# Jingliang-Duan/DSAC-v2

Measured on AMD Instinct MI355X. Metric: DSAC-T gradient steps/sec, batch=256 Humanoid (obs376/act17), higher is better.
Workload: dtype f32

## Files before the change

### dsac-v2_amd/csrc/dsact_chain.h

```cpp
#pragma once
#include "dsact_kernels.h"

namespace dsact {

#ifndef DSACT_TILE_NAP
#define DSACT_TILE_NAP 24
#endif
constexpr int kChMaxL = 4;
#ifndef DSACT_KPD
#define DSACT_KPD 16
#endif
constexpr int kPD = DSACT_KPD;

#ifdef DSACT_TIMELINE
#define CTL(buf, k) do { if ((buf) && threadIdx.x == 0 && blockIdx.x < 1024) (buf)[blockIdx.x * 16 + (k)] = (long long)__builtin_readcyclecounter(); } while (0)
#define CTLR(buf, k) do { if ((buf) && threadIdx.x == 0 && blockIdx.x < 1024) (buf)[blockIdx.x * 16 + (k)] = (long long)__builtin_amdgcn_s_memrealtime(); } while (0)
#define CTLV(buf, k, v) do { if ((buf) && threadIdx.x == 0 && blockIdx.x < 1024) (buf)[blockIdx.x * 16 + (k)] = (long long)(v); } while (0)
#else
#define CTL(buf, k) do {} while (0)
#define CTLR(buf, k) do {} while (0)
#define CTLV(buf, k, v) do {} while (0)
#endif


struct WStr { f32x4 b[kPD]; };

__device__ __forceinline__ void stream_prologue(WStr& ws, const float* cur, int s_lo, int lane4) {
#pragma unroll
  for (int u = 0; u < kPD; ++u) ws.b[u] = gload4(cur + (size_t)(s_lo + u) * 256 + lane4);
}

template <int RG>
__device__ __forceinline__ void gemm44_seg(WStr& ws, const float* cur, int s_lo, int s_hi, const float* nxt, int nxt_s0,
                                           bool has_nxt, const float* lds, int xs, int ld, int lane4, f32x4 (&acc)[RG][2]) {
  f32x4 a0[RG], a1[RG];
#pragma unroll
  for (int g = 0; g < RG; ++g) a0[g] = *(const f32x4*)(lds + xs + 4 * g * ld + 4 * s_lo);
  for (int s0 = s_lo; s0 < s_hi; s0 += kPD) {
    const float* src = s0 + kPD < s_hi ? cur + (size_t)(s0 + kPD) * 256
                                       : (has_nxt ? nxt + (size_t)nxt_s0 * 256 : cur + (size_t)s_lo * 256);
#pragma unroll
    for (int u = 0; u < kPD; ++u) {
      const int s = s0 + u;
#pragma unroll
      for (int g = 0; g < RG; ++g) {
        if (u & 1) a0[g] = *(const f32x4*)(lds + xs + 4 * g * ld + 4 * (s + 1));
        else a1[g] = *(const f32x4*)(lds + xs + 4 * g * ld + 4 * (s + 1));
      }
#pragma unroll
      for (int e = 0; e < 4; ++e) {
#pragma unroll
        for (int g = 0; g < RG; ++g)
          acc[g][e & 1] = __builtin_amdgcn_mfma_f32_4x4x1f32((u & 1) ? a1[g][e] : a0[g][e], ws.b[u][e], acc[g][e & 1], 0, 0, 0);
        if (e == 1) __builtin_amdgcn_sched_barrier(0);
      }
      ws.b[u] = gload4(src + (size_t)u * 256 + lane4);
      __builtin_amdgcn_sched_barrier(0);
    }
  }
}

template <int NTO_MAX>
struct NarrowFrags { f32x4 w[NTO_MAX][4]; };

template <int NTO_MAX>
__device__ __forceinline__ void narrow_load(NarrowFrags<NTO_MAX>& f, const float* wf, int C, int nto, int wave, int lane4) {
#pragma unroll
  for (int t = 0; t < NTO_MAX; ++t) {
    if (t < nto) {
#pragma unroll
      for (int c = 0; c < 4; ++c) f.w[t][c] = gload4(wf + ((size_t)t * C + (size_t)wave * 4 + c) * 256 + lane4);
    }
  }
}
template <int NTO_MAX>
__device__ __forceinline__ void narrow_mma(const NarrowFrags<NTO_MAX>& f, int nto, int wave, float* lds, int xs, int red, int lane) {
  f32x4 a[4];
#pragma unroll
  for (int c = 0; c < 4; ++c) a[c] = *(const f32x4*)(lds + xs + 16 * (wave * 4 + c));
#pragma unroll
  for (int t = 0; t < NTO_MAX; ++t) {
    if (t < nto) {
      f32x4 acc = {0.f, 0.f, 0.f, 0.f};
#pragma unroll
      for (int c = 0; c < 4; ++c)
#pragma unroll
        for (int e = 0; e < 4; ++e) acc = __builtin_amdgcn_mfma_f32_16x16x4f32(f.w[t][c][e], a[c][e], acc, 0, 0, 0);
      *(f32x4*)(lds + red + ((wave * NTO_MAX + t) * 64 + lane) * 4) = acc;
    }
  }
}
template <int NTO_MAX, int NW>
__device__ __forceinline__ float narrow_get(const float* lds, int red, int m, int n) {
  const int t = n >> 4, ln = (((n & 15) >> 2) << 4) + m, e = n & 3;
  float s = lds[red + ((0 * NTO_MAX + t) * 64 + ln) * 4 + e];
#pragma unroll
  for (int w = 1; w < NW; ++w) s += lds[red + ((w * NTO_MAX + t) * 64 + ln) * 4 + e];
  return s;
}

template <int TPR>
__device__ __forceinline__ float rowN_sum(float v) {
  v += dpp_mov<0xB1>(v);
  v += dpp_mov<0x4E>(v);
  if (TPR >= 8) v += dpp_mov<0x141>(v);
  if (TPR >= 16) v += dpp_mov<0x140>(v);
  if (TPR >= 32) { float a, b; swap16(v, a, b); v = a + b; }
  if (TPR >= 64) { float a, b; swap32(v, a, b); v = a + b; }
  return v;
}

__device__ __forceinline__ bool chain_decode(int b, int n_units, int n_slices, int& unit, int& slice) {
  const int rep = n_units >= 5 ? 1 : (n_units >= 3 ? 2 : (n_units == 2 ? 4 : 8));
  const int xcd = b & 7, rnd = b >> 3;
  if (xcd >= n_units * rep) return false;
  unit = xcd % n_units;
  slice = rnd * rep + xcd / n_units;
  return slice < n_slices;
}
inline int chain_grid(int n_units, int n_slices) {
  const int rep = n_units >= 5 ? 1 : (n_units >= 3 ? 2 : (n_units == 2 ? 4 : 8));
  return 8 * ((n_slices + rep - 1) / rep);
}
struct XcdMap { int unit[8], base[8], stride[8]; };
inline XcdMap xcd_map_uniform(int n_units) {
  XcdMap m;
  const int rep = n_units >= 5 ? 1 : (n_units >= 3 ? 2 : (n_units == 2 ? 4 : 8));
  for (int x = 0; x < 8; ++x) {
    const bool on = x < n_units * rep;
    m.unit[x] = on ? x % n_units : -1; m.base[x] = on ? x / n_units : 0; m.stride[x] = rep;
  }
  return m;
}
inline XcdMap xcd_map_shares(int n_units, const int* share) {
  XcdMap m;
  int x = 0;
  for (int u = 0; u < n_units; ++u)
    for (int k = 0; k < share[u] && x < 8; ++k, ++x) { m.unit[x] = u; m.base[x] = k; m.stride[x] = share[u]; }
  for (; x < 8; ++x) { m.unit[x] = -1; m.base[x] = 0; m.stride[x] = 1; }
// ... 365 lines not shown
  int s_obs, s_act;
  int v1_stats;
  const float* act_scale; const float* act_center; float lo_ls, hi_ls;
  long long* timeline;
  int* spin_timeout;
  int debug_withhold;
  const long long* tagp;
  int tpad;
  int x0_lds;
};


__device__ __forceinline__ void stores_acked_barrier() {
  asm volatile("s_waitcnt vmcnt(0) lgkmcnt(0)\n\ts_barrier" ::: "memory");
}
__device__ __forceinline__ void chain_publish(int* flag, int value = 1) {
  if (!flag) return;
  stores_acked_barrier();
  if (threadIdx.x == 0) __hip_atomic_store(flag, value, __ATOMIC_RELAXED, __HIP_MEMORY_SCOPE_AGENT);
}
__device__ __forceinline__ void chain_wait(const int* f0, const int* f1, int* timeout) {
  if (threadIdx.x == 0) {
    int spins = 0;
    for (;;) {
      const int a0 = f0 ? __hip_atomic_load(f0, __ATOMIC_RELAXED, __HIP_MEMORY_SCOPE_AGENT) : 1;
      const int a1 = f1 ? __hip_atomic_load(f1, __ATOMIC_RELAXED, __HIP_MEMORY_SCOPE_AGENT) : 1;
      if (a0 && a1) break;
      if (++spins > (1 << 17)) { if (timeout) *timeout = 1; break; }
      __builtin_amdgcn_s_sleep(16);
    }
  }
  __syncthreads();
}

constexpr int kArriveStride = 64;
__device__ __forceinline__ void pack_store4(float* p, const f32x4& v, int agent) {
  if (agent) asm volatile("global_store_dwordx4 %0, %1, off sc1" : : "v"(p), "v"(v) : "memory");
  else nt_store4(p, v);
}
__device__ __forceinline__ void hand_store(float* p, float v, int agent) {
  if (agent) st_agent(p, v); else *p = v;
}
__device__ __forceinline__ void chain_arrive(int* cnt) {
  if (!cnt) return;
  stores_acked_barrier();
  if (threadIdx.x < 8) __hip_atomic_fetch_add(cnt + threadIdx.x * kArriveStride, 1, __ATOMIC_RELAXED, __HIP_MEMORY_SCOPE_AGENT);
}
struct ArriveWait {
  const int* cnt; int need; int* timeout;
  long long* tl = nullptr;
  int quick = 0;
  __device__ __forceinline__ void operator()() const {
    if (threadIdx.x == 0) {
      const int* c = cnt + ((int)blockIdx.x & 7) * kArriveStride;
      int spins = 0;
      while (__hip_atomic_load(c, __ATOMIC_RELAXED, __HIP_MEMORY_SCOPE_AGENT) < need) {
        if (++spins > (1 << 17)) { if (timeout) *timeout = 1; break; }
        if (quick) __builtin_amdgcn_s_sleep(4); else __builtin_amdgcn_s_sleep(DSACT_TILE_NAP);
      }
    }
    asm volatile("s_barrier" ::: "memory");
    CTLR(tl, 13);
  }
};

__device__ __forceinline__ bool fwd_decode(const FwdArgs& a, int b, int& unit, int& slice) {
  const int x = b & 7;
  unit = a.map.unit[x];
  if (unit < 0) return false;
  slice = a.map.base[x] + a.map.stride[x] * (b >> 3);
  return slice < a.u[unit].n_slices;
}
inline int fwd_grid(const FwdArgs& a) {
  int rounds = 0;
  for (int x = 0; x < 8; ++x) {
    if (a.map.unit[x] < 0) continue;
    const int n = a.u[a.map.unit[x]].n_slices - a.map.base[x];
    const int r = n > 0 ? (n + a.map.stride[x] - 1) / a.map.stride[x] : 0;
    rounds = r > rounds ? r : rounds;
  }
  return 8 * rounds;
}

template <int NW, int RG, bool GA = false, typename AT = FwdArgs, typename UT = FwdUnit, bool WARM = false>
__device__ __forceinline__ void chain_fwd_body(const AT& a, const UT& u, int unit, int slice, float* lds, int warm_idx = 0, int warm_cnt = 0) {
  constexpr int W = 64 * NW, SH = W / 4, R = 4 * RG, NTHR = 64 * NW, TPR = NTHR / R;
  int* const done_flag = (u.done && !(a.debug_withhold && unit == 0 && slice == 0)) ? u.done + slice : nullptr;
  const int tid = threadIdx.x, lane = tid & 63;
  const int wave = __builtin_amdgcn_readfirstlane(tid >> 6);
  const int lane4 = lane * 4;
  const int n = 64 * wave + lane;
  const int row0 = slice * R;
  const int L = a.L, F = a.F, A = a.A;
  const int S0 = a.s_obs + u.s_act;
  const int head = u.head & HEAD_KIND, twin = u.head & (HEAD_TWIN_FIRST | HEAD_TWIN_SECOND);
  const int c_out = ((u.head >> 8) & 0xff) ? ((u.head >> 8) & 0xff) : W / 16;
  const int oact = GA ? head_out_act(u.head) : 0;
  const ChainLds S = chain_lds(4 * (a.s_obs + a.s_act), W, R);
  const int xin = S.off_in, red = S.off_red;
  CTL(a.timeline, 0);
  CTLR(a.timeline, 14);
  const bool do_obs = u.seg != SEG_ACT_FROM_SAVED;
  const bool do_act = u.seg != SEG_OBS_ONLY && u.s_act > 0;
  WStr ws;
  const float* w0 = u.wf[0] + (size_t)wave * (S0 + a.tpad) * 256;
  stream_prologue(ws, w0, do_obs ? 0 : a.s_obs, lane4);
  constexpr int NWARM = 4;
  float wt[NWARM] = {0.f, 0.f, 0.f, 0.f};
  if (WARM) {
    const int n0 = NW * S0 * 8, nh = NW * SH * 8;
    const int nhead = head == HEAD_NONE ? 0 : (head == HEAD_POLICY ? (2 * A + 15) >> 4 : 1) * (W / 16) * 8;
    const int total = warm_cnt > 0 ? n0 + (L - 1) * nh + nhead : 0;
    const int share = (total + warm_cnt - 1) / (warm_cnt > 0 ? warm_cnt : 1);
    const int lo = warm_idx * share, hi = lo + share < total ? lo + share : total;
    const float* wb[kChMaxL + 1];
#pragma unroll
    for (int l = 0; l <= kChMaxL; ++l) wb[l] = u.wf[l <= L ? l : L];
#pragma unroll
    for (int q = 0; q < NWARM; ++q) {
      int i = lo + tid + q * NTHR;
      i = i < hi ? i : lo;
      const float* base = wb[0];
      int off = i;
#pragma unroll
      for (int l = 1; l <= kChMaxL; ++l) {
        const int start = n0 + (l - 1) * nh;
        const bool in = l <= L && i >= start;
        base = in ? wb[l] : base;
        off = in ? i - start : off;
      }
      wt[q] = *(const __attribute__((address_space(1))) float*)(base + (size_t)off * 32);
    }
    __builtin_amdgcn_sched_barrier(0);
  }
  float bq[kChMaxL];
#pragma unroll
  for (int l = 0; l < kChMaxL; ++l) bq[l] = u.bias[l < L ? l : 0][n];
  const int mr = tid / TPR, jr = tid % TPR;
  constexpr int NQ = (32 + TPR - 1) / TPR;
  float pre_eps[NQ], pre_bmu[NQ], pre_braw[NQ], pre_s[NQ], pre_c[NQ];
#pragma unroll
  for (int q = 0; q < NQ; ++q) { pre_eps[q] = 0.f; pre_bmu[q] = 0.f; pre_braw[q] = 0.f; pre_s[q] = 1.f; pre_c[q] = 0.f; }
  if (head == HEAD_POLICY) {
#pragma unroll
    for (int q = 0; q < NQ; ++q) {
      const int d = jr + q * TPR;
      if (d < A) {
        pre_eps[q] = u.eps[(size_t)(row0 + mr) * A + d];
        pre_bmu[q] = u.bias[L][d]; pre_braw[q] = u.bias[L][A + d];
        pre_s[q] = a.act_scale[d]; pre_c[q] = a.act_center[d];
      }
    }
  } else if (head == HEAD_Q && jr == 0) {
    pre_bmu[0] = u.bias[L][0]; pre_braw[0] = u.bias[L][1];
  }
  const bool pairs_in = (u.late_wait & HW_PAIRS_IN) != 0, pairs_out = (u.late_wait & HW_PAIRS_OUT) != 0;
  const unsigned tag = (pairs_in || pairs_out) ? (unsigned)(*a.tagp) + 1u : 0u;
  const bool head_wait = (u.late_wait & HW_HEAD) != 0;
  const int* const flag0 = (pairs_in || head_wait) ? nullptr : u.wait0;
  const bool waits = flag0 || u.wait1 || pairs_in;
  const bool late = waits && (u.late_wait & HW_LATE) && u.seg != SEG_ACT_FROM_SAVED && u.s_act > 0;
  if ((flag0 || u.wait1) && !late)
    chain_wait(flag0 ? flag0 + row0 / u.wait_rows0 : nullptr, u.wait1 ? u.wait1 + row0 / u.wait_rows1 : nullptr, a.spin_timeout);
  f32x4 zi[RG];
  if (u.seg == SEG_ACT_FROM_SAVED) {
#pragma unroll
    for (int g = 0; g < RG; ++g)
#pragma unroll
      for (int r = 0; r < 4; ++r) zi[g][r] = ld_agent(u.zinit + (size_t)(row0 + 4 * g + r) * W + n);
  }
  auto stage_act = [&]() {
    const int Fp = 4 * a.s_obs;
    if (pairs_in) {
      const unsigned long long* hp = (const unsigned long long*)u.wait0;
      const int per_row = 4 * u.s_act;
      for (int e = tid; e < R * per_row; e += NTHR) {
        const int r = e / per_row, k = e % per_row;
        float v = 0.0f;
        if (k < A) {
          const unsigned long long* src = hp + (size_t)(row0 + r) * 32 + k;
          unsigned long long pv = __hip_atomic_load(src, __ATOMIC_RELAXED, __HIP_MEMORY_SCOPE_AGENT);
          int spins = 0;
          while ((unsigned)(pv >> 32) != tag) {
            if (++spins > (1 << 17)) { if (a.spin_timeout) *a.spin_timeout = 1; break; }
            __builtin_amdgcn_s_sleep(8);
            pv = __hip_atomic_load(src, __ATOMIC_RELAXED, __HIP_MEMORY_SCOPE_AGENT);
          }
          v = __builtin_bit_cast(float, (unsigned)pv);
        }
        lds[xin + r * S.ld_in + Fp + k] = v;
      }
      return;
    }
    const int aq = u.s_act, total = R * aq;
    for (int e = tid; e < total; e += NTHR) {
      const int r = e / aq, k = (e % aq) * 4;
      f32x4 v = {0.f, 0.f, 0.f, 0.f};
      const float* s = u.x + (size_t)(row0 + r) * a.ldx + F + k;
      for (int c = 0; c < 4; ++c) if (k + c < A) v[c] = ld_agent(s + c);
      *(f32x4*)(lds + xin + r * S.ld_in + Fp + k) = v;
    }
  };
  {
    const int Fp = 4 * a.s_obs;
    if (do_obs) {
      const int fq = Fp >> 2, total = R * fq;
      for (int e0 = tid; e0 < total; e0 += 4 * NTHR) {
        f32x4 v[4];
#pragma unroll
        for (int q = 0; q < 4; ++q) {
          const int e = e0 + q * NTHR;
          const int r = e < total ? e / fq : 0, k = e < total ? (e % fq) * 4 : 0;
          const float* s = u.x + (size_t)(row0 + r) * a.ldx + (k + 3 < F ? k : 0);
          v[q] = *(const f32x4u*)s;
        }
#pragma unroll
        for (int q = 0; q < 4; ++q) {
          const int e = e0 + q * NTHR;
          if (e < total) {
            const int r = e / fq, k = (e % fq) * 4;
            f32x4 o = v[q];
            if (k + 3 >= F) {
              const float* s = u.x + (size_t)(row0 + r) * a.ldx;
              for (int c = 0; c < 4; ++c) o[c] = k + c < F ? s[k + c] : 0.0f;
            }
            *(f32x4*)(lds + xin + r * S.ld_in + k) = o;
          }
        }
      }
    }
    if (do_act && !late) stage_act();
  }
  f32x4 acc[RG][2];
#pragma unroll
  for (int g = 0; g < RG; ++g) { acc[g][0] = f32x4{0.f, 0.f, 0.f, 0.f}; acc[g][1] = acc[g][0]; }
  if (u.seg == SEG_ACT_FROM_SAVED) {
#pragma unroll
    for (int g = 0; g < RG; ++g) acc[g][0] = zi[g];
  }
  lds_barrier();
  CTL(a.timeline, 1);
  if (u.x0t) {
    const int K0 = F + (do_act ? A : 0);
    for (int e = tid; e < K0 * RG; e += NTHR) {
      const int k = e / RG, g4 = e % RG;
      const int kk = k < F ? k : 4 * a.s_obs + (k - F);
      f32x4 v;
#pragma unroll
      for (int r = 0; r < 4; ++r) v[r] = lds[xin + (4 * g4 + r) * S.ld_in + kk];
      nt_store4(u.x0t + pk_index(k, row0 + 4 * g4, a.Cb), v);
    }
  }
  const int xs_in = xin + (lane & 3) * S.ld_in;
  const bool more = L > 1;
  const float* w1 = u.wf[more ? 1 : 0] + (size_t)wave * (more ? SH + a.tpad : S0 + a.tpad) * 256;
  if (do_obs) {
    const bool into_act = do_act;
    gemm44_seg<RG>(ws, w0, 0, a.s_obs, into_act ? w0 : w1, into_act ? a.s_obs : 0, into_act || (more && u.seg != SEG_OBS_ONLY),
                   lds, xs_in, S.ld_in, lane4, acc);
    if (u.zsave) {
#pragma unroll
      for (int g = 0; g < RG; ++g) {
        const f32x4 v = acc[g][0] + acc[g][1];
#pragma unroll
        for (int r = 0; r < 4; ++r) st_agent(u.zsave + (size_t)(row0 + 4 * g + r) * W + n, v[r]);
      }
      if (u.zdone) chain_publish(u.zdone + slice);
    }
    CTL(a.timeline, 2);
    if (WARM) {
      const float wsum = (wt[0] + wt[1]) + (wt[2] + wt[3]);
      asm volatile("" : : "v"(wsum));
    }
    if (u.seg == SEG_OBS_ONLY) { CTLR(a.timeline, 15); chain_publish(done_flag); return; }
    if (u.seg == SEG_FULL_SPLIT) {
#pragma unroll
      for (int g = 0; g < RG; ++g) { acc[g][0] = acc[g][0] + acc[g][1]; acc[g][1] = f32x4{0.f, 0.f, 0.f, 0.f}; }
    }
  }
  if (late) {
    if (flag0 || u.wait1)
      chain_wait(flag0 ? flag0 + row0 / u.wait_rows0 : nullptr, u.wait1 ? u.wait1 + row0 / u.wait_rows1 : nullptr, a.spin_timeout);
    stage_act();
    lds_barrier();
  }
  if (do_act) gemm44_seg<RG>(ws, w0, a.s_obs, S0, w1, 0, more, lds, xs_in, S.ld_in, lane4, acc);
  CTL(a.timeline, 3);
  NarrowFrags<4> hf;
  const int nto = head == HEAD_POLICY ? (2 * A + 15) >> 4 : 1;
  for (int l = 0; l < L; ++l) {
    if (l == L - 1 && head != HEAD_NONE) narrow_load<4>(hf, u.wf[L], c_out, nto, wave, lane4);
    const int hn = (l & 1) ? S.off_h1 : S.off_h0;
    const float bl = l == 0 ? bq[0] : l == 1 ? bq[1] : l == 2 ? bq[2] : bq[3];
#pragma unroll
    for (int g = 0; g < RG; ++g) {
      const f32x4 z = acc[g][0] + acc[g][1] + bl;
      f32x4 hv, gd;
      if (GA) act4(u.act, z, hv, gd); else gelu4(z, hv, gd);
#pragma unroll
      for (int r = 0; r < 4; ++r) lds[hn + (4 * g + r) * S.ld_h + n] = hv[r];
      if (u.H[l]) nt_store4(u.H[l] + pk_index(n, row0 + 4 * g, a.Cb), hv);
      if (u.G[l]) nt_store4(u.G[l] + pk_index(n, row0 + 4 * g, a.Cb), gd);
      acc[g][0] = f32x4{0.f, 0.f, 0.f, 0.f}; acc[g][1] = acc[g][0];
    }
    lds_barrier();
    CTL(a.timeline, 4 + 2 * l);
    if (l + 1 < L) {
      const float* wc = u.wf[l + 1] + (size_t)wave * (SH + a.tpad) * 256;
      const bool has_nxt = l + 2 < L;
      const float* wn = u.wf[has_nxt ? l + 2 : l + 1] + (size_t)wave * (SH + a.tpad) * 256;
      gemm44_seg<RG>(ws, wc, 0, SH, wn, 0, has_nxt, lds, hn + (lane & 3) * S.ld_h, S.ld_h, lane4, acc);
      CTL(a.timeline, 5 + 2 * l);
    }
  }
  if (head == HEAD_NONE) { CTLR(a.timeline, 15); chain_publish(done_flag); return; }
  const int hl = ((L - 1) & 1) ? S.off_h1 : S.off_h0;
  narrow_mma<4>(hf, nto, wave, lds, hl + ((lane & 15) & (R - 1)) * S.ld_h + 4 * (lane >> 4), red, lane);
  lds_barrier();
  CTL(a.timeline, 12);
  float* const carry = lds + S.off_carry;
  if (twin == HEAD_TWIN_FIRST) {
    for (int e = tid; e < R * 16 * nto; e += NTHR) {
      const int mm = e / (16 * nto), o = e % (16 * nto);
      const float v = narrow_get<4, NW>(lds, red, mm, o);
      if (u.qout) st_agent(u.qout + (size_t)(row0 + mm) * 64 + o, v);
      else carry[mm * 64 + o] = v;
    }
    CTLR(a.timeline, 15);
    if (u.qout) chain_publish(done_flag);
    return;
  }
  const bool add_carry = twin == HEAD_TWIN_SECOND;
  if (head_wait) {
    chain_wait(u.wait0 + row0 / u.wait_rows0, nullptr, a.spin_timeout);
    for (int e = tid; e < R * 16 * nto; e += NTHR) {
      const int mm = e / (16 * nto), o = e % (16 * nto);
      carry[mm * 64 + o] = ld_agent(u.zinit + (size_t)(row0 + mm) * 64 + o);
    }
    lds_barrier();
  }
  const int m = mr, j = jr;
  const int r = row0 + m;
  if (head == HEAD_Q) {
    if (j == 0) {
      float mean = narrow_get<4, NW>(lds, red, m, 0), raw = narrow_get<4, NW>(lds, red, m, 1);
      if (add_carry) { mean += carry[m * 64]; raw += carry[m * 64 + 1]; }
      mean += pre_bmu[0]; raw += pre_braw[0];
      float sgm = 1.0f;
      if (GA && oact) { mean = out_act_fwd(oact, mean); raw = out_act_fwd(oact, raw); sgm = out_act_grad_y(oact, raw); }
      u.qout[2 * r] = mean; u.qout[2 * r + 1] = raw;
      if (u.qstd) { u.qstd[2 * r] = softplus(raw); u.qstd[2 * r + 1] = softplus_grad(raw) * sgm; }
    }
    CTL(a.timeline, 13);
    CTLR(a.timeline, 15);
    chain_publish(done_flag);
    return;
  }
  float lp = 0.f, s_tanh = 0.f, s_sig = 0.f;
#pragma unroll
  for (int q = 0; q < NQ; ++q) {
    const int d = j + q * TPR;
    if (d >= A) break;
    float mu = narrow_get<4, NW>(lds, red, m, d), raw = narrow_get<4, NW>(lds, red, m, A + d);
    if (add_carry) { mu += carry[m * 64 + d]; raw += carry[m * 64 + A + d]; }
    mu += pre_bmu[q]; raw += pre_braw[q];
    if (GA && oact) { mu = out_act_fwd(oact, mu); if (!(u.head & HEAD_STD_PLAIN)) raw = out_act_fwd(oact, raw); }
    const TanhGaussFwd f = tanh_gauss_fwd(mu, raw, pre_eps[q], pre_s[q], pre_c[q], a.lo_ls, a.hi_ls);
    lp += f.lp;
    st_agent(u.xact + (size_t)r * a.ldx + F + d, f.a);
    if (pairs_out) {
      if (!(a.debug_withhold && unit == 0 && slice == 0))
        __hip_atomic_store((unsigned long long*)u.xact2 + (size_t)r * 32 + d,
                           ((unsigned long long)tag << 32) | (unsigned long long)__builtin_bit_cast(unsigned, f.a), __ATOMIC_RELAXED, __HIP_MEMORY_SCOPE_AGENT);
    } else if (u.xact2) st_agent(u.xact2 + (size_t)r * a.ldx + F + d, f.a);
    u.logits[(size_t)r * 2 * A + d] = mu;
    u.logits[(size_t)r * 2 * A + A + d] = raw;
    if (!a.v1_stats) { s_tanh += tanhf(mu); s_sig += f.sigma; }
    else {
      if (d == 0) s_tanh += tanhf(mu);
      if (A >= 2) { if (d == 1) s_sig += mu; } else s_sig += f.sigma;
    }
  }
  lp = rowN_sum<TPR>(lp);
  if (j == 0) u.logp[r] = lp;
  CTL(a.timeline, 13);
  if (u.part_heads) {
    s_tanh = rowN_sum<TPR>(s_tanh); s_sig = rowN_sum<TPR>(s_sig);
    float* sc = lds + S.off_sc;
    if (j == 0) { sc[2 * m] = s_tanh; sc[2 * m + 1] = s_sig; }
    lds_barrier();
    if (tid < RG) {
      float t0 = 0.f, t1 = 0.f;
      for (int rr = 0; rr < 4; ++rr) { t0 += sc[2 * (4 * tid + rr)]; t1 += sc[2 * (4 * tid + rr) + 1]; }
      u.part_heads[2 * (RG * slice + tid)] = t0;
      u.part_heads[2 * (RG * slice + tid) + 1] = t1;
    }
  }
  CTLR(a.timeline, 15);
  chain_publish(done_flag);
}

template <int NW, int RG, bool GA = false>
__global__ void __launch_bounds__(64 * NW, RG >= 4 ? 1 : 2) k_chain_fwd(FwdArgs a) {
  extern __shared__ __attribute__((aligned(16))) float lds[];
  int unit, slice;
  if (!fwd_decode(a, (int)blockIdx.x, unit, slice)) return;
  chain_fwd_body<NW, RG, GA>(a, a.u[unit], unit, slice, lds);
}

struct Fwd2Args { FwdArgs A, B; int n_a; };
static_assert(sizeof(Fwd2Args) <= 4096, "kernel arguments are limited to 4 KB");
template <int NW, bool GA = false>
__global__ void __launch_bounds__(64 * NW, 2) k_chain_fwd2(Fwd2Args a) {
  extern __shared__ __attribute__((aligned(16))) float lds[];
  const bool in_a = (int)blockIdx.x < a.n_a;
  const FwdArgs& f = in_a ? a.A : a.B;
  int unit, slice;
  if (!fwd_decode(f, in_a ? (int)blockIdx.x : (int)blockIdx.x - a.n_a, unit, slice)) return;
  if (f.u[unit].rg == 1) chain_fwd_body<NW, 1, GA>(f, f.u[unit], unit, slice, lds);
  else chain_fwd_body<NW, 2, GA>(f, f.u[unit], unit, slice, lds);
}

constexpr int kPipeUnits = 16;
constexpr int kPipeMaxBlocks = 1536;
struct PipeFwd {
  FwdArgs c;
  FwdUnit u[kPipeUnits];
  int n_blocks;
  DevState* book_st; StepHyper book_hp; int* book_cnt; int book_ncnt;
  int blk[kPipeMaxBlocks];
  int warm[kPipeMaxBlocks];
};
constexpr int kPipeRoleBook = 13;
__device__ __forceinline__ void pipe_book(const __attribute__((address_space(4))) PipeFwd* p) {
  if (threadIdx.x != 0) return;
  DevState* st = (DevState*)p->book_st;
  StepHyper hp;
  hp.delay_update = p->book_hp.delay_update; hp.lr_q = p->book_hp.lr_q; hp.lr_pi = p->book_hp.lr_pi; hp.lr_alpha = p->book_hp.lr_alpha;
  hp.beta1 = p->book_hp.beta1; hp.beta2 = p->book_hp.beta2;
  prologue_duties(st, st->it_next, 1, hp);
  int* c = (int*)p->book_cnt;
  for (int i = 0; i < p->book_ncnt; ++i) c[i * kArriveStride] = 0;
}
template <int NW, bool GA = false>
__global__ void __launch_bounds__(64 * NW, 2) k_chain_fwdp(const PipeFwd* __restrict__ pd) {
  extern __shared__ __attribute__((aligned(16))) float lds[];
  typedef __attribute__((address_space(4))) const PipeFwd KP;
  KP* p = (KP*)(unsigned long long)pd;
  const int code = p->blk[blockIdx.x];
  if (code < 0) return;
  const int unit = code >> 16, slice = code & 0xffff;
  if (unit == kPipeRoleBook) { pipe_book(p); return; }
#ifdef DSACT_TIMELINE
  if (p->c.timeline && threadIdx.x == 0 && blockIdx.x < 512) p->c.timeline[blockIdx.x * 16 + 11] = unit + 1;
#endif
  const int wm = p->warm[blockIdx.x];
  typedef __attribute__((address_space(4))) const FwdArgs KA;
  typedef __attribute__((address_space(4))) const FwdUnit KU;
  if (p->u[unit].rg == 1) chain_fwd_body<NW, 1, GA, KA, KU, true>(p->c, p->u[unit], unit, slice, lds, wm >> 16, wm & 0xffff);
  else chain_fwd_body<NW, 2, GA, KA, KU, true>(p->c, p->u[unit], unit, slice, lds, wm >> 16, wm & 0xffff);
}

template <int NW, bool GA = false>
__global__ void __launch_bounds__(64 * NW, 2) k_chain_fwdt(const PipeFwd* __restrict__ pd) {
  extern __shared__ __attribute__((aligned(16))) float lds[];
  typedef __attribute__((address_space(4))) const PipeFwd KP;
  KP* p = (KP*)(unsigned long long)pd;
  const int code = p->blk[blockIdx.x];
  if (code < 0) return;
  const int unit = code >> 16, slice = code & 0xffff;
  typedef __attribute__((address_space(4))) const FwdArgs KA;
  typedef __attribute__((address_space(4))) const FwdUnit KU;
  const int nt = ((p->u[unit].head & HEAD_TWIN_FIRST) && !p->u[unit].qout) ? 2 : 1;
#pragma nounroll
  for (int t = 0; t < nt; ++t) {
    if (t) lds_barrier();
    if (p->u[unit + t].rg == 1) chain_fwd_body<NW, 1, GA, KA, KU, false>(p->c, p->u[unit + t], unit + t, slice, lds);
    else chain_fwd_body<NW, 2, GA, KA, KU, false>(p->c, p->u[unit + t], unit + t, slice, lds);
  }
}

template <int NTHR>
__device__ __forceinline__ void std_column_sums(const float* p1, const float* p2, int B, int tid, float& s1, float& s2) {
  if (B <= NTHR) {
    if (tid < B) { s1 += p1[2 * tid]; s2 += p2[2 * tid]; }
    return;
  }
  for (int r0 = tid; r0 < B; r0 += 4 * NTHR) {
    float v1[4], v2[4];
#pragma unroll
    for (int q = 0; q < 4; ++q) {
      const int r = r0 + q * NTHR;
      const int rc = r < B ? r : tid;
      v1[q] = p1[2 * rc]; v2[q] = p2[2 * rc];
    }
#pragma unroll
    for (int q = 0; q < 4; ++q) {
      const bool ok = r0 + q * NTHR < B;
      s1 += ok ? v1[q] : 0.0f; s2 += ok ? v2[q] : 0.0f;
    }
  }
}

struct BwdQUnit {
  const float* wb[kChMaxL];
  const float* wout;
  const float* G[kChMaxL];
  float* dZ[kChMaxL];
  float* dout;
  float* doutT;
  const float* w1at; float* dA;
  int which;
  int trunk;
  float* dz0row;
  unsigned long long* dA_pairs;
};
struct BwdQTail {
  int n_units, n_slices;
  int B, A, L, Cb;
  const float* qout_c[2]; const float* qstd_c[2]; const float* qout_t[2]; const float* qout_p[2];
  const float* rew; const float* done; const float* logp2; const float* logp_new; const float* z5; const float* z6;
  const float* log_alpha;
  float* part_loss; float* grads_tail; const DevState* st;
  float inv_B, inv_Bg; const float* std_sums;
  int auto_alpha; float alpha_fixed, gamma, tau_b, one_minus_tau_b;
  int n_chain_blocks;
  long long* timeline;
  RideArgs ride;
  int* flags_reset; int n_flags;
  int v1; float td_bound; int v1_bound;
  int ldo;
  int c1at;
  int ldz0;
  int q_out_act;
  int* arrive;
  int debug_withhold;
  const long long* tagp;
};
template <int NU>
struct BwdQArgsN : BwdQTail {
  BwdQUnit u[NU];
};
typedef BwdQArgsN<8> BwdQArgs;
constexpr int kBqtCntInts = 3 * 8 * 64;

template <int W, int R, int NTHR>
__device__ __forceinline__ void store_dz0_rows(float* dst, int ldz0, int row0, const float* lds_rows, int ld_h) {
  const int tid = threadIdx.x;
  for (int e = tid; e < R * W; e += NTHR) {
    const int r = e / W, c = e - r * W;
    dst[(size_t)(row0 + r) * ldz0 + c] = lds_rows[r * ld_h + c];
  }
}

template <int NW, int RG, bool MRG = false, typename QA = BwdQArgs>
__device__ __forceinline__ void bwd_q_body(const QA& a, int block, float* lds) {
  if (a.flags_reset && threadIdx.x == 0)
    for (int i = block; i < a.n_flags; i += a.n_chain_blocks) a.flags_reset[i] = 0;
  int unit, slice;
  if (!chain_decode(block, a.n_units, a.n_slices, unit, slice)) return;
  constexpr int W = 64 * NW, SH = W / 4, R = 4 * RG, NTHR = 64 * NW, TPR = NTHR / R;
// ... 61 lines not shown
  const float tq = rew + nd * a.gamma * (qn - alpha * lp2);
  const float tqs = rew + nd * a.gamma * (qs - alpha * lp2);
  const CriticTerm c1 = critic_term(q1, std1, ms1, tq, tqs);
  const CriticTerm c2 = critic_term(q2, std2, ms2, tq, tqs);
  const float wq1 = q1p < q2p ? 1.0f : (q1p > q2p ? 0.0f : 0.5f);
  float d0, d1;
  if (u.which == 0) { d0 = c1.dq * a.inv_B; d1 = c1.dstd * a.inv_B * sg1; }
  else if (u.which == 1) { d0 = c2.dq * a.inv_B; d1 = c2.dstd * a.inv_B * sg2; }
  else if (u.which == 2) { d0 = -wq1 * a.inv_B; d1 = 0.0f; }
  else { d0 = -(1.0f - wq1) * a.inv_B; d1 = 0.0f; }
  if (a.q_out_act)
    d0 *= out_act_grad_y(a.q_out_act, u.which == 0 ? q1 : u.which == 1 ? q2 : u.which == 2 ? q1p : q2p);
  float v1_loss = 0.f;
  if (a.v1) {
    const float qs1 = q1n + z5 * std1n;
    const float tq1 = rew + nd * a.gamma * (qs1 - alpha * lp2);
    const float tqb = q1 + clampf(tq1 - q1, -a.td_bound, a.td_bound);
    const float sd = fmaxf(std1, 0.0f);
    float dq = -(tq1 - q1) / (sd * sd + 0.1f);
    const float e = q1 - tqb;
    float dstd = -((e * e - sd * sd) / (sd * sd * sd + 0.1f));
    v1_loss = dq * q1 + dstd * std1;
    if (!a.v1_bound) {
      const float d = tq1 - q1, var = std1 * std1;
      dq = -d / var;
      dstd = 1.0f / std1 - (d * d) / (var * std1);
      v1_loss = (d * d) / (2.0f * var) + logf(std1) + kLogSqrt2Pi;
    }
    if (u.which == 0) { d0 = dq * a.inv_B; d1 = dstd * a.inv_B * sg1; }
    else { d0 = -a.inv_B; d1 = 0.0f; }
  }
  if (j == 0) {
    sc[16 + 2 * m] = d0; sc[16 + 2 * m + 1] = d1;
    if (lead) { u.dout[2 * r] = d0; u.dout[2 * r + 1] = d1; }
    if (lead && u.doutT) { hand_store(u.doutT + pk_index(0, r, a.Cb), d0, agent); hand_store(u.doutT + pk_index(1, r, a.Cb), d1, agent); }
    if (!lead) {
    } else if (u.which == 0 && a.v1) {
      float* pl = a.part_loss + (size_t)r * kLossPart;
      pl[0] = v1_loss; pl[1] = 0.f; pl[2] = q1; pl[3] = 0.f; pl[4] = std1; pl[5] = 0.f;
      pl[6] = alpha * lpn - q1p;
      pl[7] = lpn;
      pl[8] = r == 0 ? alpha : 0.0f;
      pl[9] = 0.0f; pl[10] = std1; pl[11] = std1;
      if (r == 0) { hand_store(a.grads_tail, 0.f, merged); hand_store(a.grads_tail + 1, 0.f, merged); }
    } else if (u.which == 0) {
      float* pl = a.part_loss + (size_t)r * kLossPart;
      pl[0] = c1.loss; pl[1] = c2.loss; pl[2] = q1; pl[3] = q2; pl[4] = std1; pl[5] = std2;
      pl[6] = alpha * lpn - fminf(q1p, q2p);
      pl[7] = lpn;
      pl[8] = r == 0 ? alpha : 0.0f;
      pl[9] = 0.0f; pl[10] = std1; pl[11] = std2;
      if (r == 0) { hand_store(a.grads_tail, ms1, merged); hand_store(a.grads_tail + 1, ms2, merged); }
    }
  }
  lds_barrier();
#pragma unroll
  for (int g = 0; g < RG; ++g) {
    f32x4 ov;
#pragma unroll
    for (int rr = 0; rr < 4; ++rr) ov[rr] = (sc[16 + 2 * (4 * g + rr)] * wo0 + sc[16 + 2 * (4 * g + rr) + 1] * wo1) * gl[g][rr];
#pragma unroll
    for (int rr = 0; rr < 4; ++rr) lds[S.off_h0 + (4 * g + rr) * S.ld_h + n] = ov[rr];
    pack_store4(u.dZ[L - 1] + pk_index(n, row0 + 4 * g, a.Cb), ov, agent);
  }
  NarrowFrags<2> af;
  const int nta = (a.A + 15) >> 4;
  if (u.w1at && L == 1 && !MRG) narrow_load<2>(af, u.w1at, c1at, nta, wave, lane4);
  if (arr && L == 1) chain_arrive(arr);
  else lds_barrier();
  if (u.dz0row && L == 1) store_dz0_rows<W, R, NTHR>(u.dz0row, a.ldz0, row0, lds + S.off_h0, S.ld_h);
  CTL(a.timeline, 2);
  f32x4 acc[RG][2];
  int cur = 0;
  for (int l = L - 1; l >= 1; --l) {
#pragma unroll
    for (int g = 0; g < RG; ++g) { acc[g][0] = f32x4{0.f, 0.f, 0.f, 0.f}; acc[g][1] = acc[g][0]; }
    f32x4 gq[RG];
#pragma unroll
    for (int g = 0; g < RG; ++g) gq[g] = gload4(u.G[l - 1] + pk_index(n, row0 + 4 * g, a.Cb));
    const bool has_nxt = l > 1;
    const float* wl = u.wb[l] + (size_t)wave * SH * 256;
    const float* wn = u.wb[has_nxt ? l - 1 : l] + (size_t)wave * SH * 256;
    const int xop = (cur ? S.off_h1 : S.off_h0) + (lane & 3) * S.ld_h;
    gemm44_seg<RG>(ws, wl, 0, SH, wn, 0, has_nxt, lds, xop, S.ld_h, lane4, acc);
    CTL(a.timeline, 3 + 2 * (L - 1 - l));
    if (l == 1 && u.w1at && !MRG) narrow_load<2>(af, u.w1at, c1at, nta, wave, lane4);
    const int hn = cur ? S.off_h0 : S.off_h1;
#pragma unroll
    for (int g = 0; g < RG; ++g) {
      const f32x4 dz = (acc[g][0] + acc[g][1]) * gq[g];
#pragma unroll
      for (int rr = 0; rr < 4; ++rr) lds[hn + (4 * g + rr) * S.ld_h + n] = dz[rr];
      pack_store4(u.dZ[l - 1] + pk_index(n, row0 + 4 * g, a.Cb), dz, agent);
    }
    cur ^= 1;
    if (arr && l == 1) chain_arrive(arr);
    else lds_barrier();
    if (u.dz0row && l == 1) store_dz0_rows<W, R, NTHR>(u.dz0row, a.ldz0, row0, lds + hn, S.ld_h);
    CTL(a.timeline, 4 + 2 * (L - 1 - l));
  }
  if (!u.w1at) { CTLR(a.timeline, 15); return; }
  if (MRG) narrow_load<2>(af, u.w1at, c1at, nta, wave, lane4);
  narrow_mma<2>(af, nta, wave, lds, (cur ? S.off_h1 : S.off_h0) + ((lane & 15) & (R - 1)) * S.ld_h + 4 * (lane >> 4), red, lane);
  lds_barrier();
  const unsigned ptag = (MRG && u.dA_pairs) ? (unsigned)(*a.tagp) + 1u : 0u;
  for (int d = j; d < 16 * nta; d += TPR) {
    const float v = d < a.A ? narrow_get<2, NW>(lds, red, m, d) : 0.0f;
    u.dA[(size_t)r * 32 + d] = v;
    if (MRG && u.dA_pairs)
      __hip_atomic_store(u.dA_pairs + (size_t)r * 32 + d, ((unsigned long long)ptag << 32) | (unsigned long long)__builtin_bit_cast(unsigned, v),
                         __ATOMIC_RELAXED, __HIP_MEMORY_SCOPE_AGENT);
  }
  CTL(a.timeline, 12);
  CTLR(a.timeline, 15);
}

template <int NW, int RG>
__global__ void __launch_bounds__(256) k_chain_bwd_q(BwdQArgs a) {
  extern __shared__ __attribute__((aligned(16))) float lds[];
  if ((int)blockIdx.x >= a.n_chain_blocks) { loss_rider(a.ride); return; }
  bwd_q_body<NW, RG>(a, (int)blockIdx.x, lds);
}

struct BwdPiArgs {
  int n_trunks;
  const float* woutT1; const float* wb1[kChMaxL]; const float* G1[kChMaxL]; float* dZ1[kChMaxL];
  const float* dA2[2];
  float* dz0row; int ldz0;
  const float* dA[2];
  const float* logits_pi; const float* eps_new; const float* log_alpha;
  const float* woutT; int SoT;
  const float* wb[kChMaxL];
  const float* G[kChMaxL];
  float* dZ[kChMaxL];
  float* dout_pi; float* d_new_act;
  float* dout_piT;
  int n_slices, B, A, L, Cb;
  float inv_B; int auto_alpha; float alpha_fixed;
  int pi_out_act, pi_out_n;
  const float* act_scale; float lo_ls, hi_ls;
  const float* part_loss; int n_part; float target_entropy; float* grad_log_alpha;
  int n_chain_blocks;
  int tile0, n_extra;
  int merge_dw, pi_tile0, n_pi_tiles, finalize;
  int* cnt_pi; int* spin_timeout;
  const unsigned long long* dA_pairs[2]; const long long* tagp;
  int debug_withhold;
  long long* timeline;
  Dw2Args dw;
};

__device__ __forceinline__ void bwd_pi_alpha_grad(const BwdPiArgs& a, int lane) {
  float s = 0.f;
  for (int r0 = 0; r0 < a.n_part; r0 += 64) {
    const int rr = r0 + lane;
    s += rr < a.n_part ? a.part_loss[(size_t)rr * kLossPart + 7] : 0.f;
  }
  s = wave_sum(s);
  if (lane == 0) a.grad_log_alpha[0] = a.auto_alpha ? -(s * a.inv_B + a.target_entropy) : 0.0f;
}

template <int NW, int RG>
__device__ __forceinline__ void bwd_pi_body(const BwdPiArgs& a, int slice, float* lds, int trunk = 0) {
  constexpr int W = 64 * NW, SH = W / 4, R = 4 * RG, NTHR = 64 * NW, TPR = NTHR / R;
  const int tid = threadIdx.x;
  if (slice >= a.n_slices || tid >= NTHR) return;
  const bool lead = trunk == 0;
  const float* const* const t_wb = trunk ? a.wb1 : a.wb;
  const float* const* const t_G = trunk ? a.G1 : a.G;
  float* const* const t_dZ = trunk ? a.dZ1 : a.dZ;
  float* const dz0row = a.dz0row ? a.dz0row + trunk * W : nullptr;
  const int lane = tid & 63;
  const int wave = __builtin_amdgcn_readfirstlane(tid >> 6);
  const int lane4 = lane * 4;
  const int n = 64 * wave + lane;
  const int row0 = slice * R;
  const int L = a.L, A = a.A;
  const ChainLds S = chain_lds(4 * a.SoT, W, R);
  float* xdo = lds + S.off_in;
  CTL(a.timeline, 0);
  CTLR(a.timeline, 14);
  WStr ws;
  const float* wo = (trunk ? a.woutT1 : a.woutT) + (size_t)wave * a.SoT * 256;
  stream_prologue(ws, wo, 0, lane4);
  const int m = tid / TPR, j = tid % TPR;
// ... 210 lines not shown
  int* spin_timeout;
  const float* logp_new; int n_part; float target_entropy; float* grad_log_alpha; int finalize;
};
static_assert(sizeof(BwdQpArgs) <= 4096, "kernel arguments are limited to 4 KB");

template <int NW, int RGQ, int RGP>
__global__ void __launch_bounds__(256, DSACT_BQT_OCC) k_chain_bwd_qpt(BwdQpArgs a) {
  extern __shared__ __attribute__((aligned(16))) float lds[];
  int idx = (int)blockIdx.x;
  if (idx < a.q.n_chain_blocks) { bwd_q_body<NW, RGQ, true, BwdQArgsN<4> >(a.q, idx, lds); return; }
  idx -= a.q.n_chain_blocks;
  if (idx < a.pi.n_chain_blocks) { CTLV(a.pi.timeline, 11, 5); bwd_pi_body<NW, RGP>(a.pi, idx, lds); return; }
  idx -= a.pi.n_chain_blocks;
  if (idx < a.n_riders) { loss_rider(a.q.ride); return; }
  idx -= a.n_riders;
  const int L = a.q.L;
  const int n_pol_blocks = xcd_chunk_grid(a.pi.n_pi_tiles);
  if (idx < a.n_tile_blocks + n_pol_blocks) {
    int t;
    const int* cnt;
    int need;
    if (idx < a.n_tile_blocks) {
      t = ((const __attribute__((address_space(4))) int*)(unsigned long long)a.tile_tab)[idx];
      if (t < 0) return;
      int pi = 0;
#pragma unroll
      for (int q = 0; q + 1 < kMaxDwProb; ++q)
        if (q + 1 < a.pi.dw.n_prob && t >= a.pi.dw.tile_ends[q]) pi = q + 1;
      cnt = a.q.arrive + (pi / (L + 1)) * 8 * kArriveStride;
      need = a.need_c;
      CTLV(a.q.timeline, 11, 10);
    } else {
      if (!xcd_chunk(idx - a.n_tile_blocks, a.pi.n_pi_tiles, t)) return;
      t += a.pi.pi_tile0;
      cnt = a.pi.cnt_pi;
      need = a.pi.n_slices;
      CTLV(a.q.timeline, 11, 11);
    }
    CTLR(a.q.timeline, 14);
    dw2_tile<2, ArriveWait>(a.pi.dw, t, lds, ArriveWait{cnt, need, a.spin_timeout, a.q.timeline});
    CTLR(a.q.timeline, 15);
    return;
  }
  ArriveWait{a.pi.cnt_pi, a.pi.n_slices, a.spin_timeout}();
  ArriveWait{a.q.arrive, a.need_c, a.spin_timeout}();
  ArriveWait{a.q.arrive + 8 * kArriveStride, a.need_c, a.spin_timeout}();
  if (threadIdx.x < 64) {
    const int lane = (int)threadIdx.x;
    float s = 0.f;
    for (int r0 = 0; r0 < a.n_part; r0 += 64) {
      const int rr = r0 + lane;
      s += rr < a.n_part ? a.logp_new[rr] : 0.f;
    }
    s = wave_sum(s);
    if (lane == 0) {
      a.grad_log_alpha[0] = a.q.auto_alpha ? -(s * a.q.inv_B + a.target_entropy) : 0.0f;
      if (a.finalize) finalize_update(a.pi.dw.fo);
    }
  }
}

constexpr int kPipeRoleBwdPi = 14, kPipeRoleTile = 15;
template <int NW, bool GA = false>
__global__ void __launch_bounds__(256, 2) k_chain_fwdpb(const PipeFwd* __restrict__ pd, BwdPiArgs bp, int bp_rg) {
  extern __shared__ __attribute__((aligned(16))) float lds[];
  typedef __attribute__((address_space(4))) const PipeFwd KP;
  KP* p = (KP*)(unsigned long long)pd;
  const int code = p->blk[blockIdx.x];
  if (code < 0) return;
  const int unit = code >> 16, slice = code & 0xffff;
#ifdef DSACT_TIMELINE
  if (p->c.timeline && threadIdx.x == 0 && blockIdx.x < 512) p->c.timeline[blockIdx.x * 16 + 11] = unit + 1;
#endif
  if (unit == kPipeRoleBwdPi) {
    if (bp_rg == 1) bwd_pi_body<NW, 1>(bp, slice, lds); else bwd_pi_body<NW, 2>(bp, slice, lds);
    return;
  }
  if (unit == kPipeRoleTile) {
    dw2_tile<2, ArriveWait>(bp.dw, bp.pi_tile0 + slice, lds, ArriveWait{pi_tile_counter(bp, bp.pi_tile0 + slice), bp.n_slices, bp.spin_timeout});
    return;
  }
  if (unit == kPipeRoleBook) { pipe_book(p); return; }
  if ((int)threadIdx.x >= 64 * NW) return;
  const int wm = p->warm[blockIdx.x];
  typedef __attribute__((address_space(4))) const FwdArgs KA;
  typedef __attribute__((address_space(4))) const FwdUnit KU;
  if (p->u[unit].rg == 1) chain_fwd_body<NW, 1, GA, KA, KU, true>(p->c, p->u[unit], unit, slice, lds, wm >> 16, wm & 0xffff);
  else chain_fwd_body<NW, 2, GA, KA, KU, true>(p->c, p->u[unit], unit, slice, lds, wm >> 16, wm & 0xffff);
}

}
```

Before: 17970.

## Prefetch narrow head weights via GEMM stream tail; drop L2 warm-up reads

In the backward chain, the last layer's weight stream now spends its final prefetch slots loading the w1at narrow-head fragments instead of wrapping back to the current layer. The merged path then reads those fragments from registers rather than issuing a separate narrow_load after the GEMM, which hides that load latency behind the MFMA loop. The change also removes the WARM cache-warming loads from the forward body and the per-block warm table in PipeFwd. The tail path depends on kPD >= 8 and on an indexing scheme that assumes at most two narrow tiles. Dropping the warm-up may cost extra cold L2 misses on weights in later stages.

```diff
diff --git a/dsac-v2_amd/csrc/dsact_chain.h b/dsac-v2_amd/csrc/dsact_chain.h
--- a/dsac-v2_amd/csrc/dsact_chain.h
+++ b/dsac-v2_amd/csrc/dsact_chain.h
@@ -30,15 +30,20 @@
   for (int u = 0; u < kPD; ++u) ws.b[u] = gload4(cur + (size_t)(s_lo + u) * 256 + lane4);
 }
 
-template <int RG>
+template <int RG, bool TAIL = false>
 __device__ __forceinline__ void gemm44_seg(WStr& ws, const float* cur, int s_lo, int s_hi, const float* nxt, int nxt_s0,
-                                           bool has_nxt, const float* lds, int xs, int ld, int lane4, f32x4 (&acc)[RG][2]) {
+                                           bool has_nxt, const float* lds, int xs, int ld, int lane4, f32x4 (&acc)[RG][2],
+                                           const float* tail = nullptr, int tail_c = 0, int tail_nt = 0) {
+  static_assert(!TAIL || kPD >= 8, "the tail takes 8 slots of the stream");
   f32x4 a0[RG], a1[RG];
 #pragma unroll
   for (int g = 0; g < RG; ++g) a0[g] = *(const f32x4*)(lds + xs + 4 * g * ld + 4 * s_lo);
   for (int s0 = s_lo; s0 < s_hi; s0 += kPD) {
     const float* src = s0 + kPD < s_hi ? cur + (size_t)(s0 + kPD) * 256
                                        : (has_nxt ? nxt + (size_t)nxt_s0 * 256 : cur + (size_t)s_lo * 256);
+    const bool at_tail = TAIL && tail != nullptr && !has_nxt && !(s0 + kPD < s_hi);
+    const float* src8 = at_tail ? tail : src;
+    const int tq = at_tail ? (tail_nt > 1 ? tail_c : 0) : 4;
 #pragma unroll
     for (int u = 0; u < kPD; ++u) {
       const int s = s0 + u;
@@ -54,7 +59,8 @@
           acc[g][e & 1] = __builtin_amdgcn_mfma_f32_4x4x1f32((u & 1) ? a1[g][e] : a0[g][e], ws.b[u][e], acc[g][e & 1], 0, 0, 0);
         if (e == 1) __builtin_amdgcn_sched_barrier(0);
       }
-      ws.b[u] = gload4(src + (size_t)u * 256 + lane4);
+      if (TAIL && u < 8) ws.b[u] = gload4(src8 + (size_t)((u >> 2) * tq + (u & 3)) * 256 + lane4);
+      else ws.b[u] = gload4(src + (size_t)u * 256 + lane4);
       __builtin_amdgcn_sched_barrier(0);
     }
   }
@@ -586,8 +592,8 @@
   return 8 * rounds;
 }
 
-template <int NW, int RG, bool GA = false, typename AT = FwdArgs, typename UT = FwdUnit, bool WARM = false>
-__device__ __forceinline__ void chain_fwd_body(const AT& a, const UT& u, int unit, int slice, float* lds, int warm_idx = 0, int warm_cnt = 0) {
+template <int NW, int RG, bool GA = false, typename AT = FwdArgs, typename UT = FwdUnit>
+__device__ __forceinline__ void chain_fwd_body(const AT& a, const UT& u, int unit, int slice, float* lds) {
   constexpr int W = 64 * NW, SH = W / 4, R = 4 * RG, NTHR = 64 * NW, TPR = NTHR / R;
   int* const done_flag = (u.done && !(a.debug_withhold && unit == 0 && slice == 0)) ? u.done + slice : nullptr;
   const int tid = threadIdx.x, lane = tid & 63;
@@ -609,34 +615,6 @@
   WStr ws;
   const float* w0 = u.wf[0] + (size_t)wave * (S0 + a.tpad) * 256;
   stream_prologue(ws, w0, do_obs ? 0 : a.s_obs, lane4);
-  constexpr int NWARM = 4;
-  float wt[NWARM] = {0.f, 0.f, 0.f, 0.f};
-  if (WARM) {
-    const int n0 = NW * S0 * 8, nh = NW * SH * 8;
-    const int nhead = head == HEAD_NONE ? 0 : (head == HEAD_POLICY ? (2 * A + 15) >> 4 : 1) * (W / 16) * 8;
-    const int total = warm_cnt > 0 ? n0 + (L - 1) * nh + nhead : 0;
-    const int share = (total + warm_cnt - 1) / (warm_cnt > 0 ? warm_cnt : 1);
-    const int lo = warm_idx * share, hi = lo + share < total ? lo + share : total;
-    const float* wb[kChMaxL + 1];
-#pragma unroll
-    for (int l = 0; l <= kChMaxL; ++l) wb[l] = u.wf[l <= L ? l : L];
-#pragma unroll
-    for (int q = 0; q < NWARM; ++q) {
-      int i = lo + tid + q * NTHR;
-      i = i < hi ? i : lo;
-      const float* base = wb[0];
-      int off = i;
-#pragma unroll
-      for (int l = 1; l <= kChMaxL; ++l) {
-        const int start = n0 + (l - 1) * nh;
-        const bool in = l <= L && i >= start;
-        base = in ? wb[l] : base;
-        off = in ? i - start : off;
-      }
-      wt[q] = *(const __attribute__((address_space(1))) float*)(base + (size_t)off * 32);
-    }
-    __builtin_amdgcn_sched_barrier(0);
-  }
   float bq[kChMaxL];
 #pragma unroll
   for (int l = 0; l < kChMaxL; ++l) bq[l] = u.bias[l < L ? l : 0][n];
@@ -772,10 +750,6 @@
       if (u.zdone) chain_publish(u.zdone + slice);
     }
     CTL(a.timeline, 2);
-    if (WARM) {
-      const float wsum = (wt[0] + wt[1]) + (wt[2] + wt[3]);
-      asm volatile("" : : "v"(wsum));
-    }
     if (u.seg == SEG_OBS_ONLY) { CTLR(a.timeline, 15); chain_publish(done_flag); return; }
     if (u.seg == SEG_FULL_SPLIT) {
 #pragma unroll
@@ -933,7 +907,6 @@
   int n_blocks;
   DevState* book_st; StepHyper book_hp; int* book_cnt; int book_ncnt;
   int blk[kPipeMaxBlocks];
-  int warm[kPipeMaxBlocks];
 };
 constexpr int kPipeRoleBook = 13;
 __device__ __forceinline__ void pipe_book(const __attribute__((address_space(4))) PipeFwd* p) {
@@ -958,11 +931,10 @@
 #ifdef DSACT_TIMELINE
   if (p->c.timeline && threadIdx.x == 0 && blockIdx.x < 512) p->c.timeline[blockIdx.x * 16 + 11] = unit + 1;
 #endif
-  const int wm = p->warm[blockIdx.x];
   typedef __attribute__((address_space(4))) const FwdArgs KA;
   typedef __attribute__((address_space(4))) const FwdUnit KU;
-  if (p->u[unit].rg == 1) chain_fwd_body<NW, 1, GA, KA, KU, true>(p->c, p->u[unit], unit, slice, lds, wm >> 16, wm & 0xffff);
-  else chain_fwd_body<NW, 2, GA, KA, KU, true>(p->c, p->u[unit], unit, slice, lds, wm >> 16, wm & 0xffff);
+  if (p->u[unit].rg == 1) chain_fwd_body<NW, 1, GA, KA, KU>(p->c, p->u[unit], unit, slice, lds);
+  else chain_fwd_body<NW, 2, GA, KA, KU>(p->c, p->u[unit], unit, slice, lds);
 }
 
 template <int NW, bool GA = false>
@@ -979,8 +951,8 @@
 #pragma nounroll
   for (int t = 0; t < nt; ++t) {
     if (t) lds_barrier();
-    if (p->u[unit + t].rg == 1) chain_fwd_body<NW, 1, GA, KA, KU, false>(p->c, p->u[unit + t], unit + t, slice, lds);
-    else chain_fwd_body<NW, 2, GA, KA, KU, false>(p->c, p->u[unit + t], unit + t, slice, lds);
+    if (p->u[unit + t].rg == 1) chain_fwd_body<NW, 1, GA, KA, KU>(p->c, p->u[unit + t], unit + t, slice, lds);
+    else chain_fwd_body<NW, 2, GA, KA, KU>(p->c, p->u[unit + t], unit + t, slice, lds);
   }
 }
 
@@ -1208,7 +1180,8 @@
     const float* wl = u.wb[l] + (size_t)wave * SH * 256;
     const float* wn = u.wb[has_nxt ? l - 1 : l] + (size_t)wave * SH * 256;
     const int xop = (cur ? S.off_h1 : S.off_h0) + (lane & 3) * S.ld_h;
-    gemm44_seg<RG>(ws, wl, 0, SH, wn, 0, has_nxt, lds, xop, S.ld_h, lane4, acc);
+    gemm44_seg<RG, MRG>(ws, wl, 0, SH, wn, 0, has_nxt, lds, xop, S.ld_h, lane4, acc,
+                        u.w1at ? u.w1at + (size_t)wave * 4 * 256 : nullptr, c1at, nta);
     CTL(a.timeline, 3 + 2 * (L - 1 - l));
     if (l == 1 && u.w1at && !MRG) narrow_load<2>(af, u.w1at, c1at, nta, wave, lane4);
     const int hn = cur ? S.off_h0 : S.off_h1;
@@ -1226,7 +1199,14 @@
     CTL(a.timeline, 4 + 2 * (L - 1 - l));
   }
   if (!u.w1at) { CTLR(a.timeline, 15); return; }
-  if (MRG) narrow_load<2>(af, u.w1at, c1at, nta, wave, lane4);
+  if (MRG) {
+    if (L > 1) {
+#pragma unroll
+      for (int t = 0; t < 2; ++t)
+#pragma unroll
+        for (int c = 0; c < 4; ++c) af.w[t][c] = ws.b[4 * t + c];
+    } else narrow_load<2>(af, u.w1at, c1at, nta, wave, lane4);
+  }
   narrow_mma<2>(af, nta, wave, lds, (cur ? S.off_h1 : S.off_h0) + ((lane & 15) & (R - 1)) * S.ld_h + 4 * (lane >> 4), red, lane);
   lds_barrier();
   const unsigned ptag = (MRG && u.dA_pairs) ? (unsigned)(*a.tagp) + 1u : 0u;
@@ -1603,11 +1583,10 @@
   }
   if (unit == kPipeRoleBook) { pipe_book(p); return; }
   if ((int)threadIdx.x >= 64 * NW) return;
-  const int wm = p->warm[blockIdx.x];
   typedef __attribute__((address_space(4))) const FwdArgs KA;
   typedef __attribute__((address_space(4))) const FwdUnit KU;
-  if (p->u[unit].rg == 1) chain_fwd_body<NW, 1, GA, KA, KU, true>(p->c, p->u[unit], unit, slice, lds, wm >> 16, wm & 0xffff);
-  else chain_fwd_body<NW, 2, GA, KA, KU, true>(p->c, p->u[unit], unit, slice, lds, wm >> 16, wm & 0xffff);
-}
-
-}
+  if (p->u[unit].rg == 1) chain_fwd_body<NW, 1, GA, KA, KU>(p->c, p->u[unit], unit, slice, lds);
+  else chain_fwd_body<NW, 2, GA, KA, KU>(p->c, p->u[unit], unit, slice, lds);
+}
+
+}
```

After: 18310 (median of 6 runs). 1.02x the previous value.
